# sutro-sh/sutro

Hardware: AMD Instinct MI355X
Metric: output_tokens_per_sec (higher is better)
Workload: dtype bf16; 1 GPU; model=qwen-3-32b, global_batch=2048, seq_len=256, parallelism=dp1, prompt_len=128, priming=seeded

## Files before the change

csrc/bindings.cpp:

```cpp
#include <torch/extension.h>

#include <hip/hip_runtime.h>
#include <c10/hip/HIPStream.h>

#define CHECK_CUDA(x) TORCH_CHECK((x).is_cuda(), #x " must be a GPU tensor")
#define CHECK_CONTIG(x) TORCH_CHECK((x).is_contiguous(), #x " must be contiguous")
#define CHECK_BF16(x) \
  TORCH_CHECK((x).scalar_type() == at::kBFloat16, #x " must be bf16")

static hipStream_t cur_stream() {
  return c10::hip::getCurrentHIPStream().stream();
}

extern "C" {
void sutro_rmsnorm(void*, const void*, const void*, float, long, int,
                   hipStream_t);
void sutro_fused_add_rmsnorm(void*, void*, const void*, float, long, int,
                             hipStream_t);
void sutro_silu_mul(void*, const void*, long, int, hipStream_t);
void sutro_rope_and_cache(void*, void*, const void*, const long*, const long*,
                          void*, void*, const float*, int, int, int, int, int,
                          hipStream_t);
static bool is_fp8(const torch::Tensor& t) {
  return t.scalar_type() == at::kFloat8_e4m3fn;
}
void sutro_mean_pool_normalize(float*, const void*, const int*, int, int,
                               hipStream_t);
void sutro_attn_decode(void*, const void*, const void*, const void*,
                       const int*, const int*, int, int, int, int, int, int,
                       int, float, hipStream_t);
void sutro_attn_prefill(void*, const void*, const void*, const void*,
                        const int*, const int*, const int*, const int*,
                        const int*, int, int, int, int, int, int, float,
                        hipStream_t);
void sutro_attn_decode_shared(void*, const void*, const void*, const void*,
                              const int*, const int*, int, int, int, int,
                              float, int, int, const int*, const int*, int,
                              int, float*, float*, float*, hipStream_t);
int sutro_attn_prefix_tile_rows(int, int);
void sutro_mfma32_probe(float*, const void*, const void*, hipStream_t);
void sutro_gemm_tn_launch(void*, const void*, const void*, const void*, int,
                          int, long, int, int, int, int, hipStream_t);
int sutro_gemm_tn_pipe_launch(void*, const void*, const void*, const void*,
                              int, int, long, int, int, int, hipStream_t);
void sutro_mfma16_probe(float*, const void*, const void*, hipStream_t);
void sutro_hd64_stage_probe(float*, float*, void*, const void*, const void*,
                            const void*, int, float, hipStream_t);
void sutro_qkv_prep(const void*, void*, void*, void*, const long*, const long*,
                    const float*, const void*, const void*, float, int, int,
                    int, int, int, int, int, hipStream_t);
void sutro_sampler_fused(const void*, int, const float*, const float*,
                         const int*, const float*, const unsigned int*, int,
                         long, int, int, int*, float*, hipStream_t);
void sutro_grouped_gemm(void*, const void*, const void*, const int*,
                        const int*, const int*, int, int, int, long, int,
                        int, hipStream_t);
void sutro_moe_combine(void*, const void*, const long*, const float*, int,
                       int, int, hipStream_t);
void sutro_logit_penalties(void*, int, const int*, const int*, const int*,
                           const int*, const int*, const float*, const float*,
                           const float*, const int*, const float*, int, int,
                           long, int, int, int, int, int, hipStream_t);
void sutro_quant_rows_fp8(void*, float*, const void*, const int*, int, long,
                          int, int, hipStream_t);
void sutro_grouped_gemm_fp8(void*, const void*, const float*, const void*,
                            const float*, const int*, const int*, const int*,
                            int, int, int, long, int, int, hipStream_t);
void sutro_quant_weight_mxfp4(void*, void*, const void*, long, int, int,
                              hipStream_t);
void sutro_grouped_gemm_mxfp4(void*, const void*, const float*, const void*,
                              const void*, const int*, const int*, const int*,
                              int, int, int, long, int, int, hipStream_t);
int sutro_gemm_tn_fp8_pipe_launch(void*, const void*, const float*,
                                  const void*, const float*, const void*, int,
                                  int, long, int, int, hipStream_t);
}

void rmsnorm(torch::Tensor out, torch::Tensor x, torch::Tensor w, double eps) {
  CHECK_CUDA(x); CHECK_CONTIG(x); CHECK_BF16(x);
  const long C = x.size(-1);
  const long rows = x.numel() / C;
  TORCH_CHECK(C % 8 == 0 && C <= 16384, "unsupported row size ", C);
  sutro_rmsnorm(out.data_ptr(), x.data_ptr(), w.data_ptr(), (float)eps, rows,
                (int)C, cur_stream());
}

void fused_add_rmsnorm(torch::Tensor x, torch::Tensor residual, torch::Tensor w,
                       double eps) {
  CHECK_CUDA(x); CHECK_CONTIG(x); CHECK_BF16(x); CHECK_CONTIG(residual);
  const long C = x.size(-1);
  const long rows = x.numel() / C;
  TORCH_CHECK(C % 8 == 0 && C <= 16384, "unsupported row size ", C);
  sutro_fused_add_rmsnorm(x.data_ptr(), residual.data_ptr(), w.data_ptr(),
                          (float)eps, rows, (int)C, cur_stream());
}

void silu_mul(torch::Tensor out, torch::Tensor x) {
// ... 137 lines not shown
                 is_fp8(k_cache) ? 1 : 0, cur_stream());
}

torch::Tensor gemm_tn(torch::Tensor x, torch::Tensor w,
                      c10::optional<torch::Tensor> res, long bm, long bn,
                      long swz, long xcd_swz) {
  CHECK_CUDA(x); CHECK_BF16(x); CHECK_CUDA(w); CHECK_BF16(w);
  TORCH_CHECK(x.is_contiguous() && w.is_contiguous(), "contiguous required");
  const long M = x.size(0), K = x.size(1), N = w.size(0);
  TORCH_CHECK(w.size(1) == K, "K mismatch");
  TORCH_CHECK(M % bm == 0 && K % 64 == 0, "shape not tile-divisible");
  auto out = torch::empty({M, N}, x.options());
  const void* rp = nullptr;
  if (res.has_value()) {
    CHECK_CUDA(*res); CHECK_BF16(*res);
    TORCH_CHECK(res->is_contiguous() && res->size(0) == M && res->size(1) == N,
                "res shape");
    rp = res->data_ptr();
  }
  sutro_gemm_tn_launch(out.data_ptr(), x.data_ptr(), w.data_ptr(), rp, (int)M,
                       (int)N, K, (int)bm, (int)bn, (int)swz, (int)xcd_swz,
                       cur_stream());
  return out;
}

torch::Tensor gemm_tn_pipelined(torch::Tensor x, torch::Tensor w,
                                c10::optional<torch::Tensor> res, long swz,
                                long xcd_swz) {
  CHECK_CUDA(x); CHECK_BF16(x); CHECK_CUDA(w); CHECK_BF16(w);
  TORCH_CHECK(x.dim() == 2 && w.dim() == 2, "x and w must be 2-d");
  TORCH_CHECK(x.is_contiguous() && w.is_contiguous(), "contiguous required");
  const long M = x.size(0), K = x.size(1), N = w.size(0);
  TORCH_CHECK(w.size(1) == K, "K mismatch");
  TORCH_CHECK(M >= 1 && N >= 1 && K >= 64 && K % 64 == 0,
              "shape not tile-divisible");
  TORCH_CHECK(M < (1L << 31) && N < (1L << 31), "M/N too large");
  TORCH_CHECK(swz >= 0 && swz <= 2, "swz must be 0, 1 or 2");
  auto out = torch::empty({M, N}, x.options());
  const void* rp = nullptr;
  if (res.has_value()) {
    CHECK_CUDA(*res); CHECK_BF16(*res);
    TORCH_CHECK(res->is_contiguous() && res->dim() == 2 &&
                res->size(0) == M && res->size(1) == N, "res shape");
    rp = res->data_ptr();
  }
  const int e = sutro_gemm_tn_pipe_launch(
      out.data_ptr(), x.data_ptr(), w.data_ptr(), rp, (int)M, (int)N, K,
      rp ? 1 : 0, (int)swz, (int)xcd_swz, cur_stream());
  TORCH_CHECK(e == 0, "gemm_tn_pipelined launch setup failed: ", e);
  return out;
}

torch::Tensor gemm_gate_up_silu(torch::Tensor x, torch::Tensor w, long swz,
                                long xcd_swz) {
  CHECK_CUDA(x); CHECK_BF16(x); CHECK_CUDA(w); CHECK_BF16(w);
  TORCH_CHECK(x.dim() == 2 && w.dim() == 2, "x and w must be 2-d");
  TORCH_CHECK(x.is_contiguous() && w.is_contiguous(), "contiguous required");
  const long M = x.size(0), K = x.size(1), N = w.size(0);
  TORCH_CHECK(w.size(1) == K, "K mismatch");
  TORCH_CHECK(M >= 1 && K >= 64 && K % 64 == 0, "shape not tile-divisible");
  TORCH_CHECK(N >= 256 && N % 256 == 0,
              "gate_up rows must be 2*I with I % 128 == 0");
  TORCH_CHECK(M < (1L << 31) && N < (1L << 31), "M/N too large");
  TORCH_CHECK(swz >= 0 && swz <= 2, "swz must be 0, 1 or 2");
  auto out = torch::empty({M, N / 2}, x.options());
  const int e = sutro_gemm_tn_pipe_launch(
      out.data_ptr(), x.data_ptr(), w.data_ptr(), nullptr, (int)M, (int)N, K,
      2, (int)swz, (int)xcd_swz, cur_stream());
  TORCH_CHECK(e == 0, "gemm_gate_up_silu launch setup failed: ", e);
  return out;
}

static void check_fp8_gemm_args(const torch::Tensor& a_q,
                                const torch::Tensor& a_scale,
                                const torch::Tensor& w_q,
                                const torch::Tensor& w_scale) {
  CHECK_CUDA(a_q); CHECK_CONTIG(a_q); CHECK_CUDA(w_q); CHECK_CONTIG(w_q);
  TORCH_CHECK(is_fp8(a_q) && is_fp8(w_q), "a_q, w_q must be float8_e4m3fn");
  CHECK_CUDA(a_scale); CHECK_CONTIG(a_scale);
  CHECK_CUDA(w_scale); CHECK_CONTIG(w_scale);
  TORCH_CHECK(a_scale.scalar_type() == at::kFloat
              && w_scale.scalar_type() == at::kFloat, "scales must be f32");
  TORCH_CHECK(a_q.dim() == 2 && w_q.dim() == 2, "a_q and w_q must be 2-d");
  const long M = a_q.size(0), Kp = a_q.size(1), N = w_q.size(0);
  TORCH_CHECK(w_q.size(1) == Kp, "Kp mismatch");
  TORCH_CHECK(M >= 1 && Kp >= 128 && Kp % 128 == 0,
              "needs M >= 1 and Kp a positive multiple of 128 (Kp=", Kp, ")");
  TORCH_CHECK(M <= (1L << 31) - 256 && N <= (1L << 31) - 256,
              "M/N too large");
  TORCH_CHECK(a_scale.numel() == M, "a_scale must be [M]");
  TORCH_CHECK(w_scale.numel() == N, "w_scale must be [N]");
}

torch::Tensor gemm_fp8_pipelined(torch::Tensor a_q, torch::Tensor a_scale,
                                 torch::Tensor w_q, torch::Tensor w_scale,
                                 c10::optional<torch::Tensor> res,
                                 long xcd_swz) {
  check_fp8_gemm_args(a_q, a_scale, w_q, w_scale);
  const long M = a_q.size(0), Kp = a_q.size(1), N = w_q.size(0);
  TORCH_CHECK(N >= 64 && N % 64 == 0, "N must be a multiple of 64 (N=", N, ")");
  auto out = torch::empty({M, N}, a_q.options().dtype(at::kBFloat16));
  const void* rp = nullptr;
  if (res.has_value()) {
    CHECK_CUDA(*res); CHECK_BF16(*res);
    TORCH_CHECK(res->is_contiguous() && res->dim() == 2 &&
                res->size(0) == M && res->size(1) == N, "res shape");
    rp = res->data_ptr();
  }
  const int e = sutro_gemm_tn_fp8_pipe_launch(
      out.data_ptr(), a_q.data_ptr(), a_scale.data_ptr<float>(),
      w_q.data_ptr(), w_scale.data_ptr<float>(), rp, (int)M, (int)N, Kp,
      rp ? 1 : 0, (int)xcd_swz, cur_stream());
  TORCH_CHECK(e == 0, "gemm_fp8_pipelined launch setup failed: ", e);
  return out;
}

torch::Tensor gemm_fp8_gate_up_silu(torch::Tensor a_q, torch::Tensor a_scale,
                                    torch::Tensor w_q, torch::Tensor w_scale,
                                    long xcd_swz) {
  check_fp8_gemm_args(a_q, a_scale, w_q, w_scale);
  const long M = a_q.size(0), Kp = a_q.size(1), N = w_q.size(0);
// ... 322 lines not shown
  const long need = 2 * (max_hist_len + n_bias);
  const int log2_cap = need <= 2048 ? 11 : (need <= 8192 ? 13 : 14);
  sutro_logit_penalties(logits.data_ptr(), f32 ? 1 : 0,
                        row_idx.data_ptr<int>(), hist.data_ptr<int>(),
                        slot.data_ptr<int>(), hist_len.data_ptr<int>(),
                        prompt_len.data_ptr<int>(), rep.data_ptr<float>(),
                        pres.data_ptr<float>(), freq.data_ptr<float>(), btp,
                        bvp, (int)m, (int)n, v_row, (int)vl, (int)n_slots,
                        (int)lcap, (int)n_bias, log2_cap, cur_stream());
}

PYBIND11_MODULE(TORCH_EXTENSION_NAME, m) {
  m.def("rmsnorm", &rmsnorm, "RMSNorm (bf16, CDNA4)");
  m.def("fused_add_rmsnorm", &fused_add_rmsnorm, "residual+=x; x=rmsnorm");
  m.def("silu_mul", &silu_mul, "fused SwiGLU");
  m.def("rope_and_cache", &rope_and_cache, "RoPE + paged KV write");
  m.def("qkv_prep", &qkv_prep, "fused qk-norm + RoPE + KV write + q gather");
  m.def("mean_pool_normalize", &mean_pool_normalize, "varlen mean pool + L2");
  m.def("paged_attention", &paged_attention, "paged prefill+decode attention");
  m.def("paged_attention_decode_shared", &paged_attention_decode_shared,
        "decode attention, shared-prefix tiles + per-row continuation");
  m.def("prefix_tile_rows", &prefix_tile_rows,
        "rows per shared-prefix tile for a (Hq, Hk) head layout");
  m.def("mfma32_probe", &mfma32_probe, "MFMA fragment-layout probe");
  m.def("mfma16_probe", &mfma16_probe, "16x16 MFMA fragment-layout probe");
  m.def("hd64_stage_probe", &hd64_stage_probe, "D=64 decode stage dump probe");
  m.def("moe_combine", &moe_combine, "fused MoE weighted gather-combine");
  m.def("grouped_gemm", &grouped_gemm,
        "dropless MoE grouped GEMM (padded segments, static grid)");
  m.def("quant_rows_fp8", &quant_rows_fp8,
        "bf16 rows -> e4m3 codes + f32 per-row scale (K padded to 128)");
  m.def("grouped_gemm_fp8", &grouped_gemm_fp8,
        "dropless MoE grouped GEMM, e4m3 operands on the block-scaled MFMA");
  m.def("quant_weight_mxfp4", &quant_weight_mxfp4,
        "bf16 rows -> e2m1 code pairs + e8m0 scale per 32 (K padded to 128)");
  m.def("grouped_gemm_mxfp4", &grouped_gemm_mxfp4,
        "dropless MoE grouped GEMM, e4m3 x MXFP4 on the block-scaled MFMA");
  m.def("sampler_fused", &sampler_fused,
        "fused mask+temp+topk/topp+sample+logprob (radix descent, no sort)");
  m.def("logit_penalties", &logit_penalties,
        "sparse repetition/presence/frequency penalties + logit_bias "
        "(LDS hash of the row history, in place)");
  m.def("gemm_tn", &gemm_tn, "bf16 TN GEMM (MFMA, glds dbuf)",
        py::arg("x"), py::arg("w"), py::arg("res") = c10::nullopt,
        py::arg("bm") = 256, py::arg("bn") = 256, py::arg("swz") = 2,
        py::arg("xcd_swz") = 0);
  m.def("gemm_tn_pipelined", &gemm_tn_pipelined,
        "bf16 TN GEMM (MFMA, 8-phase glds pipeline, any M/N)",
        py::arg("x"), py::arg("w"), py::arg("res") = c10::nullopt,
        py::arg("swz") = 2, py::arg("xcd_swz") = 1);
  m.def("gemm_gate_up_silu", &gemm_gate_up_silu,
        "SwiGLU fused into the pipelined gate_up GEMM",
        py::arg("x"), py::arg("w"), py::arg("swz") = 2,
        py::arg("xcd_swz") = 1);
  m.def("gemm_fp8_pipelined", &gemm_fp8_pipelined,
        "e4m3 W8A8 TN GEMM (block-scaled MFMA, 8-phase glds pipeline)",
        py::arg("a_q"), py::arg("a_scale"), py::arg("w_q"),
        py::arg("w_scale"), py::arg("res") = c10::nullopt,
        py::arg("xcd_swz") = 1);
  m.def("gemm_fp8_gate_up_silu", &gemm_fp8_gate_up_silu,
        "SwiGLU fused into the pipelined e4m3 gate_up GEMM",
        py::arg("a_q"), py::arg("a_scale"), py::arg("w_q"),
        py::arg("w_scale"), py::arg("xcd_swz") = 1);
}
```

csrc/gemm_tn_pipe.hip:

```cpp
#include "common.h"

typedef s16x8 bf16x8;

namespace {

__device__ __forceinline__ f32x4 mfma16(bf16x8 a, bf16x8 b, f32x4 c) {
  return __builtin_amdgcn_mfma_f32_16x16x32_bf16(a, b, c, 0, 0, 0);
}

__device__ __forceinline__ void glds16(const char* g, char* lds) {
  __builtin_amdgcn_global_load_lds(
      (const __attribute__((address_space(1))) u32*)g,
      (__attribute__((address_space(3))) u32*)lds, 16, 0, 0);
}

template <int SWZ>
__device__ __forceinline__ u32 swz(u32 byte) {
  if (SWZ == 1) return byte ^ (((byte >> 9) & 1u) << 5);
  if (SWZ == 2) return byte ^ (((byte >> 8) & 7u) << 4);
  return byte;
}

constexpr int HT = 16384;
constexpr int KTILE_B = 65536;
constexpr int SLOT_B0 = 0, SLOT_A0 = 1, SLOT_B1 = 2, SLOT_A1 = 3;

struct Src {
  const char* p[2];
};

template <int SWZ>
__device__ __forceinline__ Src make_src(const u16* base, long row0,
                                        long rows_valid, long Kb, int wave,
                                        int lane) {
  Src s;
#pragma unroll
  for (int j = 0; j < 2; ++j) {
    const u32 b = (u32)(wave * 2 + j) * 1024u + (u32)lane * 16u;
    const u32 lb = swz<SWZ>(b);
    long row = (long)(lb >> 7);
    row = row < rows_valid ? row : rows_valid - 1;
    s.p[j] = (const char*)base + (row0 + row) * Kb + (lb & 127u);
  }
  return s;
}

__device__ __forceinline__ void stage_half(char* slot_wave, const Src& s,
                                           long koff) {
  glds16(s.p[0] + koff, slot_wave);
  glds16(s.p[1] + koff, slot_wave + 1024);
}

__device__ __forceinline__ bf16x8 lds_frag(const char* smem, u32 off) {
  return *(const bf16x8*)(smem + off);
}

}

template <int EPI, int SWZ>
__global__ __launch_bounds__(512) void gemm_tn_pipe_kernel(
    u16* __restrict__ out, const u16* __restrict__ x,
    const u16* __restrict__ w, const u16* __restrict__ res, int M, int N,
    long K, int xcd_swz) {
  extern __shared__ __attribute__((aligned(1024))) char smem[];

  const int lane = threadIdx.x & 63;
  const int wave = __builtin_amdgcn_readfirstlane(threadIdx.x >> 6);
  const int wm = wave >> 2;
  const int wn = wave & 3;

  int bid = blockIdx.x;
  if (xcd_swz) {
    const int nwg = gridDim.x;
    const int q = nwg >> 3, r = nwg & 7;
    const int xcd = bid & 7, seq = bid >> 3;
    bid = (xcd < r ? xcd * (q + 1) : r * (q + 1) + (xcd - r) * q) + seq;
  }
  const int MT = (M + 255) >> 8;
  const int m0 = (bid % MT) * 256;
  const int I = N >> 1;
  const int nt = bid / MT;
  const int nb0 = (EPI == 2) ? nt * 128 : nt * 256;
  const int nb1 = (EPI == 2) ? I + nt * 128 : nt * 256 + 128;
  const int nlim = (EPI == 2) ? I : N;

  const long Kb = K * 2;
  const long a0v = min(128, M - m0);
  const long a1v = max(1, min(128, M - m0 - 128));
  const long b0v = min(128, nlim - nb0);
  const long b1v = (EPI == 2) ? 128 : max(1, min(128, N - nb1));
  const long a1r = (M - m0 - 128 >= 1) ? m0 + 128 : m0 + a0v - 1;
  const long b1r = (EPI == 2 || N - nb1 >= 1) ? nb1 : nb0 + b0v - 1;
  const Src sB0 = make_src<SWZ>(w, nb0, b0v, Kb, wave, lane);
  const Src sA0 = make_src<SWZ>(x, m0, a0v, Kb, wave, lane);
  const Src sB1 = make_src<SWZ>(w, b1r, b1v, Kb, wave, lane);
  const Src sA1 = make_src<SWZ>(x, a1r, a1v, Kb, wave, lane);

  char* const sw = smem + wave * 2048;

  u32 aoff[2], boff[2];
#pragma unroll
  for (int kk = 0; kk < 2; ++kk) {
    const u32 kc = (u32)(kk * 4 + (lane >> 4)) * 16u;
    aoff[kk] = swz<SWZ>((u32)(wm * 64 + (lane & 15)) * 128u + kc);
    boff[kk] = swz<SWZ>((u32)(wn * 32 + (lane & 15)) * 128u + kc);
  }

  f32x4 acc[2][2][4][2];
#pragma unroll
  for (int a = 0; a < 2; ++a)
#pragma unroll
    for (int b = 0; b < 2; ++b)
#pragma unroll
      for (int i = 0; i < 4; ++i)
#pragma unroll
        for (int j = 0; j < 2; ++j) acc[a][b][i][j] = f32x4{0.f, 0.f, 0.f, 0.f};

  const int KT = (int)(K >> 6);
  const int klast = KT - 1;

  {
    const long k1 = (long)min(1, klast) * 128;
    stage_half(sw + SLOT_B0 * HT, sB0, 0);
    stage_half(sw + SLOT_A0 * HT, sA0, 0);
    stage_half(sw + SLOT_B1 * HT, sB1, 0);
    stage_half(sw + SLOT_A1 * HT, sA1, 0);
    stage_half(sw + KTILE_B + SLOT_B0 * HT, sB0, k1);
    stage_half(sw + KTILE_B + SLOT_A0 * HT, sA0, k1);
    stage_half(sw + KTILE_B + SLOT_B1 * HT, sB1, k1);
    asm volatile("s_waitcnt vmcnt(6)" ::: "memory");
    __builtin_amdgcn_s_barrier();
    if (wm == 1) __builtin_amdgcn_s_barrier();
  }

  bf16x8 fa[4][2], fb0[2][2], fb1[2][2];

#define PHASE_SYNC_MFMA(A_, B_, FB_)                                     \
  __builtin_amdgcn_sched_barrier(0);                                     \
  __builtin_amdgcn_s_barrier();                                          \
  asm volatile("s_waitcnt lgkmcnt(0)" ::: "memory");                     \
  __builtin_amdgcn_sched_barrier(0);                                     \
  __builtin_amdgcn_s_setprio(1);                                         \
  _Pragma("unroll") for (int kk = 0; kk < 2; ++kk)                       \
  _Pragma("unroll") for (int i = 0; i < 4; ++i)                          \
  _Pragma("unroll") for (int j = 0; j < 2; ++j)                          \
      acc[A_][B_][i][j] = mfma16(fa[i][kk], FB_[j][kk], acc[A_][B_][i][j]); \
  __builtin_amdgcn_s_setprio(0);                                         \
  __builtin_amdgcn_sched_barrier(0);                                     \
  __builtin_amdgcn_s_barrier();                                          \
  __builtin_amdgcn_sched_barrier(0);

#define KTILE(P)                                                         \
  {                                                                      \
    const char* cur = smem + (P) * KTILE_B;                              \
    char* nxt = sw + ((P) ^ 1) * KTILE_B;                                \
    char* own = sw + (P) * KTILE_B;                                      \
                                                                \
    _Pragma("unroll") for (int j = 0; j < 2; ++j)                        \
    _Pragma("unroll") for (int kk = 0; kk < 2; ++kk)                     \
        fb0[j][kk] = lds_frag(cur + SLOT_B0 * HT + j * 2048, boff[kk]);  \
    __builtin_amdgcn_sched_barrier(0);                                   \
    _Pragma("unroll") for (int i = 0; i < 4; ++i)                        \
    _Pragma("unroll") for (int kk = 0; kk < 2; ++kk)                     \
        fa[i][kk] = lds_frag(cur + SLOT_A0 * HT + i * 2048, aoff[kk]);   \
    __builtin_amdgcn_sched_barrier(0);                                   \
    stage_half(nxt + SLOT_A1 * HT, sA1, kn1);                            \
    __builtin_amdgcn_sched_barrier(0);                                   \
    asm volatile("s_waitcnt lgkmcnt(8)" ::: "memory");                   \
    PHASE_SYNC_MFMA(0, 0, fb0)                                           \
                                                                \
    _Pragma("unroll") for (int j = 0; j < 2; ++j)                        \
    _Pragma("unroll") for (int kk = 0; kk < 2; ++kk)                     \
        fb1[j][kk] = lds_frag(cur + SLOT_B1 * HT + j * 2048, boff[kk]);  \
    __builtin_amdgcn_sched_barrier(0);                                   \
    stage_half(own + SLOT_B0 * HT, sB0, kn2);                            \
    PHASE_SYNC_MFMA(0, 1, fb1)                                           \
                                                                \
    _Pragma("unroll") for (int i = 0; i < 4; ++i)                        \
    _Pragma("unroll") for (int kk = 0; kk < 2; ++kk)                     \
        fa[i][kk] = lds_frag(cur + SLOT_A1 * HT + i * 2048, aoff[kk]);   \
    __builtin_amdgcn_sched_barrier(0);                                   \
    stage_half(own + SLOT_A0 * HT, sA0, kn2);                            \
    PHASE_SYNC_MFMA(1, 0, fb0)                                           \
                                                                \
    stage_half(own + SLOT_B1 * HT, sB1, kn2);                            \
    __builtin_amdgcn_sched_barrier(0);                                   \
    asm volatile("s_waitcnt vmcnt(6)" ::: "memory");                     \
    PHASE_SYNC_MFMA(1, 1, fb1)                                           \
  }

  for (int t = 0; t < KT; t += 2) {
    {
      const long kn1 = (long)min(t + 1, klast) * 128;
      const long kn2 = (long)min(t + 2, klast) * 128;
      KTILE(0)
    }
    if (t + 1 < KT) {
      const long kn1 = (long)min(t + 2, klast) * 128;
      const long kn2 = (long)min(t + 3, klast) * 128;
      KTILE(1)
    }
  }
#undef KTILE
#undef PHASE_SYNC_MFMA

  asm volatile("s_waitcnt vmcnt(0)" ::: "memory");
  if (wm == 0) __builtin_amdgcn_s_barrier();

  const int drow = (lane >> 4) * 4;
  const int dcol = lane & 15;
  if (EPI == 2) {
#pragma unroll
    for (int a = 0; a < 2; ++a)
#pragma unroll
      for (int i = 0; i < 4; ++i)
#pragma unroll
        for (int j = 0; j < 2; ++j) {
          const int gn = nb0 + wn * 32 + j * 16 + dcol;
          const int gm = m0 + a * 128 + wm * 64 + i * 16 + drow;
#pragma unroll
          for (int r = 0; r < 4; ++r) {
            if (gm + r >= M) continue;
            const float gf = bf2f(f2bf(acc[a][0][i][j][r]));
            const float uf = bf2f(f2bf(acc[a][1][i][j][r]));
            const float s = gf / (1.f + __expf(-gf));
            out[(long)(gm + r) * I + gn] = f2bf(s * uf);
          }
        }
  } else {
#pragma unroll
    for (int a = 0; a < 2; ++a)
#pragma unroll
      for (int b = 0; b < 2; ++b)
#pragma unroll
        for (int i = 0; i < 4; ++i)
#pragma unroll
          for (int j = 0; j < 2; ++j) {
            const int gn = nb0 + b * 128 + wn * 32 + j * 16 + dcol;
            if (gn >= N) continue;
            const int gm = m0 + a * 128 + wm * 64 + i * 16 + drow;
#pragma unroll
            for (int r = 0; r < 4; ++r) {
              if (gm + r >= M) continue;
              const long o = (long)(gm + r) * N + gn;
              float v = acc[a][b][i][j][r];
              if (EPI == 1) v += bf2f(res[o]);
              out[o] = f2bf(v);
            }
          }
  }
}

extern "C" int sutro_gemm_tn_pipe_launch(void* out, const void* x,
                                         const void* w, const void* res,
                                         int M, int N, long K, int epi,
                                         int swz_mode, int xcd_swz,
                                         hipStream_t stream) {
  constexpr int LDS_BYTES = 2 * KTILE_B;
  const int mt = (M + 255) / 256;
  const int ntl = (epi == 2) ? (N / 2) / 128 : (N + 255) / 256;
  dim3 grid(mt * ntl), block(512);
  constexpr int MAX_DEV = 64;
  static bool attr_set[3][3][MAX_DEV];
  int dev = 0;
  const int ed = (int)hipGetDevice(&dev);
  if (ed != 0) return ed;
#define LAUNCH_1(EPI, SWZ)                                                   \
  if (epi == EPI && swz_mode == SWZ) {                                       \
    if (dev < 0 || dev >= MAX_DEV || !attr_set[EPI][SWZ][dev]) {             \
      const int e = (int)hipFuncSetAttribute(                                \
          (const void*)gemm_tn_pipe_kernel<EPI, SWZ>,                        \
          hipFuncAttributeMaxDynamicSharedMemorySize, LDS_BYTES);            \
      if (e != 0) return e;                                                  \
      if (dev >= 0 && dev < MAX_DEV) attr_set[EPI][SWZ][dev] = true;         \
    }                                                                        \
    gemm_tn_pipe_kernel<EPI, SWZ><<<grid, block, LDS_BYTES, stream>>>(       \
        (u16*)out, (const u16*)x, (const u16*)w, (const u16*)res, M, N, K,   \
        xcd_swz);                                                            \
    return 0;                                                                \
  }
#define LAUNCH(EPI) LAUNCH_1(EPI, 0) LAUNCH_1(EPI, 1) LAUNCH_1(EPI, 2)
  LAUNCH(0)
  LAUNCH(1)
  LAUNCH(2)
#undef LAUNCH
#undef LAUNCH_1
  return -1;
}
```

sutro_amd/ops/__init__.py:

```python

from __future__ import annotations

import os
from typing import Optional

import torch

from . import torch_ref

_C = None
_C_ERR: Optional[str] = None
try:
    from sutro_amd import _C as _C
except Exception as e:
    _C_ERR = f"{type(e).__name__}: {e}"


def hip_available() -> bool:
    return _C is not None


def _require_hip():
    if _C is None:
        raise RuntimeError(
            "sutro_amd HIP extension (_C) is not built but a GPU tensor was passed. "
            "Build it with `python setup.py build_ext --inplace` "
            f"(import error: {_C_ERR})"
        )
    return _C


_FORCE_REF = os.environ.get("SUTRO_AMD_FORCE_TORCH_REF", "0") == "1"


def _use_hip(t: torch.Tensor) -> bool:
    return t.is_cuda and not _FORCE_REF


def rmsnorm(x: torch.Tensor, weight: torch.Tensor, eps: float) -> torch.Tensor:
    if _use_hip(x):
        out = torch.empty_like(x)
        _require_hip().rmsnorm(out, x, weight, eps)
        return out
    return torch_ref.rmsnorm(x, weight, eps)


def fused_add_rmsnorm(x, residual, weight, eps: float):
    if _use_hip(x):
        _require_hip().fused_add_rmsnorm(x, residual, weight, eps)
        return x, residual
    return torch_ref.fused_add_rmsnorm(x, residual, weight, eps)


def silu_mul(x: torch.Tensor) -> torch.Tensor:
    if _use_hip(x):
        T, two_i = x.shape
        out = torch.empty((T, two_i // 2), dtype=x.dtype, device=x.device)
        _require_hip().silu_mul(out, x)
        return out
    return torch_ref.silu_mul(x)


GATE_UP_FUSED_RULE: dict = {
    (5120, 51200): (1152, frozenset({1536, 1664, 1792})),
}

_GATE_UP_FORCE: Optional[bool] = {"1": True, "0": False}.get(
    os.environ.get("SUTRO_GATE_UP_FUSED", ""))


def set_gate_up_fused(mode: Optional[bool]) -> None:
    global _GATE_UP_FORCE
    _GATE_UP_FORCE = mode


def gate_up_silu_qualifies(x: torch.Tensor, weight: torch.Tensor) -> bool:
    return (x.dim() == 2 and weight.dim() == 2 and x.shape[0] >= 1
            and x.dtype == torch.bfloat16 and weight.dtype == torch.bfloat16
            and x.is_contiguous() and weight.is_contiguous()
            and x.shape[1] == weight.shape[1] and x.shape[1] % 64 == 0
            and weight.shape[0] >= 256 and weight.shape[0] % 256 == 0)


def gate_up_silu(x: torch.Tensor, weight: torch.Tensor) -> torch.Tensor:
    if _use_hip(x) and gate_up_silu_qualifies(x, weight):
        if _GATE_UP_FORCE is None:
            min_m, held_back = GATE_UP_FUSED_RULE.get(
                (x.shape[1], weight.shape[0]), (None, ()))
            fused = (min_m is not None and x.shape[0] >= min_m
                     and x.shape[0] not in held_back)
        else:
            fused = _GATE_UP_FORCE
        if fused:
            return _require_hip().gemm_gate_up_silu(x, weight)
    return silu_mul(torch.nn.functional.linear(x, weight))


def fused_qkv_prep(
    qkv: torch.Tensor,
    num_heads: int, num_kv_heads: int, head_dim: int,
    positions: torch.Tensor, slot_mapping: torch.Tensor,
    k_cache: torch.Tensor, v_cache: torch.Tensor,
    cos_sin: torch.Tensor,
    q_norm_w: Optional[torch.Tensor] = None,
    k_norm_w: Optional[torch.Tensor] = None,
    eps: float = 1e-6,
) -> torch.Tensor:
    T = qkv.shape[0]
    if _use_hip(qkv):
        q_out = torch.empty((T, num_heads, head_dim), dtype=qkv.dtype,
                            device=qkv.device)
        _require_hip().qkv_prep(qkv, q_out, k_cache, v_cache, positions,
                                slot_mapping, cos_sin, q_norm_w, k_norm_w, eps)
        return q_out
    q_size = num_heads * head_dim
    kv_size = num_kv_heads * head_dim
    q, k, v = qkv.split([q_size, kv_size, kv_size], dim=-1)
    q = q.reshape(T, num_heads, head_dim).contiguous()
    k = k.reshape(T, num_kv_heads, head_dim).contiguous()
    v = v.reshape(T, num_kv_heads, head_dim).contiguous()
    if q_norm_w is not None:
        q = torch_ref.rmsnorm(q, q_norm_w, eps)
    if k_norm_w is not None:
        k = torch_ref.rmsnorm(k, k_norm_w, eps)
    q, k = torch_ref.apply_rope(q, k, positions, cos_sin)
    torch_ref.write_kv_cache(k, v, k_cache, v_cache, slot_mapping)
    return q


def rope_and_cache(
    q: torch.Tensor, k: torch.Tensor, v: torch.Tensor,
    positions: torch.Tensor, slot_mapping: torch.Tensor,
    k_cache: torch.Tensor, v_cache: torch.Tensor,
    cos_sin: torch.Tensor,
) -> torch.Tensor:
    if _use_hip(q):
        _require_hip().rope_and_cache(q, k, v, positions, slot_mapping,
                                      k_cache, v_cache, cos_sin)
        return q
    q, k = torch_ref.apply_rope(q, k, positions, cos_sin)
    torch_ref.write_kv_cache(k, v, k_cache, v_cache, slot_mapping)
    return q


_EMPTY_I32: Optional[torch.Tensor] = None


# ... 233 lines not shown
```

Before: 7492 tokens/s.

## Add grouped/banded tile ordering and persistent variant to fused SwiGLU gate_up GEMM

```diff
diff --git a/csrc/bindings.cpp b/csrc/bindings.cpp
--- a/csrc/bindings.cpp
+++ b/csrc/bindings.cpp
@@ -42,7 +42,9 @@
 void sutro_gemm_tn_launch(void*, const void*, const void*, const void*, int,
                           int, long, int, int, int, int, hipStream_t);
 int sutro_gemm_tn_pipe_launch(void*, const void*, const void*, const void*,
-                              int, int, long, int, int, int, hipStream_t);
+                              int, int, long, int, int, int, hipStream_t,
+                              int variant = 0, int group_m = 0,
+                              int num_blocks = 0, int wide = 0);
 void sutro_mfma16_probe(float*, const void*, const void*, hipStream_t);
 void sutro_hd64_stage_probe(float*, float*, void*, const void*, const void*,
                             const void*, int, float, hipStream_t);
@@ -286,7 +288,8 @@
 }
 
 torch::Tensor gemm_gate_up_silu(torch::Tensor x, torch::Tensor w, long swz,
-                                long xcd_swz) {
+                                long xcd_swz, long variant, long group_m,
+                                long num_blocks, bool wide) {
   CHECK_CUDA(x); CHECK_BF16(x); CHECK_CUDA(w); CHECK_BF16(w);
   TORCH_CHECK(x.dim() == 2 && w.dim() == 2, "x and w must be 2-d");
   TORCH_CHECK(x.is_contiguous() && w.is_contiguous(), "contiguous required");
@@ -297,10 +300,28 @@
               "gate_up rows must be 2*I with I % 128 == 0");
   TORCH_CHECK(M < (1L << 31) && N < (1L << 31), "M/N too large");
   TORCH_CHECK(swz >= 0 && swz <= 2, "swz must be 0, 1 or 2");
+  TORCH_CHECK(variant == 0 || variant == 1,
+              "variant must be 0 (one tile per block) or 1 (persistent)");
+  TORCH_CHECK(group_m > -(1L << 24) && group_m < (1L << 24),
+              "group_m out of range");
+  TORCH_CHECK(group_m >= 0 || xcd_swz != 0,
+              "the banded tile order (group_m < 0) needs xcd_swz");
+  TORCH_CHECK(num_blocks >= -1 && num_blocks <= (1L << 20),
+              "num_blocks out of range");
+  TORCH_CHECK(((M + 255) / 256) * (N / 256) < (1L << 31), "too many tiles");
+  if (variant == 1) {
+    TORCH_CHECK(K % 128 == 0 && K <= (1L << 23),
+                "the persistent gate_up kernel needs K % 128 == 0 (got K = ",
+                K, "); use variant 0");
+  } else {
+    TORCH_CHECK(num_blocks == 0 && !wide,
+                "num_blocks / wide apply to the persistent variant only");
+  }
   auto out = torch::empty({M, N / 2}, x.options());
   const int e = sutro_gemm_tn_pipe_launch(
       out.data_ptr(), x.data_ptr(), w.data_ptr(), nullptr, (int)M, (int)N, K,
-      2, (int)swz, (int)xcd_swz, cur_stream());
+      2, (int)swz, (int)xcd_swz, cur_stream(), (int)variant, (int)group_m,
+      (int)num_blocks, wide ? 1 : 0);
   TORCH_CHECK(e == 0, "gemm_gate_up_silu launch setup failed: ", e);
   return out;
 }
@@ -729,7 +750,9 @@
   m.def("gemm_gate_up_silu", &gemm_gate_up_silu,
         "SwiGLU fused into the pipelined gate_up GEMM",
         py::arg("x"), py::arg("w"), py::arg("swz") = 2,
-        py::arg("xcd_swz") = 1);
+        py::arg("xcd_swz") = 1, py::arg("variant") = 0,
+        py::arg("group_m") = 0, py::arg("num_blocks") = 0,
+        py::arg("wide") = false);
   m.def("gemm_fp8_pipelined", &gemm_fp8_pipelined,
         "e4m3 W8A8 TN GEMM (block-scaled MFMA, 8-phase glds pipeline)",
         py::arg("a_q"), py::arg("a_scale"), py::arg("w_q"),
diff --git a/csrc/gemm_tn_pipe.hip b/csrc/gemm_tn_pipe.hip
--- a/csrc/gemm_tn_pipe.hip
+++ b/csrc/gemm_tn_pipe.hip
@@ -55,85 +55,90 @@
   return *(const bf16x8*)(smem + off);
 }
 
-}
-
-template <int EPI, int SWZ>
-__global__ __launch_bounds__(512) void gemm_tn_pipe_kernel(
-    u16* __restrict__ out, const u16* __restrict__ x,
-    const u16* __restrict__ w, const u16* __restrict__ res, int M, int N,
-    long K, int xcd_swz) {
-  extern __shared__ __attribute__((aligned(1024))) char smem[];
-
-  const int lane = threadIdx.x & 63;
-  const int wave = __builtin_amdgcn_readfirstlane(threadIdx.x >> 6);
-  const int wm = wave >> 2;
-  const int wn = wave & 3;
-
-  int bid = blockIdx.x;
-  if (xcd_swz) {
-    const int nwg = gridDim.x;
-    const int q = nwg >> 3, r = nwg & 7;
-    const int xcd = bid & 7, seq = bid >> 3;
-    bid = (xcd < r ? xcd * (q + 1) : r * (q + 1) + (xcd - r) * q) + seq;
-  }
-  const int MT = (M + 255) >> 8;
-  const int m0 = (bid % MT) * 256;
-  const int I = N >> 1;
-  const int nt = bid / MT;
-  const int nb0 = (EPI == 2) ? nt * 128 : nt * 256;
-  const int nb1 = (EPI == 2) ? I + nt * 128 : nt * 256 + 128;
-  const int nlim = (EPI == 2) ? I : N;
-
-  const long Kb = K * 2;
-  const long a0v = min(128, M - m0);
-  const long a1v = max(1, min(128, M - m0 - 128));
-  const long b0v = min(128, nlim - nb0);
-  const long b1v = (EPI == 2) ? 128 : max(1, min(128, N - nb1));
+__device__ __forceinline__ void tile_mn(int tile, int MT, int NT, int group_m,
+                                        int& mt, int& nt) {
+  if (group_m <= 0 || group_m >= MT) {
+    mt = tile % MT;
+    nt = tile / MT;
+    return;
+  }
+  const int per = group_m * NT;
+  const int g = tile / per;
+  const int first = g * group_m;
+  const int gsz = min(group_m, MT - first);
+  const int local = tile - g * per;
+  mt = first + local % gsz;
+  nt = local / gsz;
+}
+
+__device__ __forceinline__ void tile_mn_banded(int xl, int i, int nx, int MT,
+                                               int NT, int group_m, int& mt,
+                                               int& nt) {
+  const int a = MT / nx, b = MT - a * nx;
+  const int whole = a * NT;
+  if (i < whole) {
+    tile_mn(i, a, NT, -group_m, mt, nt);
+    mt += a * xl;
+    return;
+  }
+  const int left = b * NT;
+  const int q = left / nx, r = left % nx;
+  const int idx =
+      (xl < r ? xl * (q + 1) : r * (q + 1) + (xl - r) * q) + (i - whole);
+  mt = nx * a + idx % b;
+  nt = idx / b;
+}
+
+struct USrc {
+  const char* base;
+  u32 o0, o1;
+};
+
+template <int SWZ>
+__device__ __forceinline__ void lane_offsets(u32& o0, u32& o1, int rows_valid,
+                                             u32 Kb, int wave, int lane) {
+  u32 o[2];
+#pragma unroll
+  for (int j = 0; j < 2; ++j) {
+    const u32 b = (u32)(wave * 2 + j) * 1024u + (u32)lane * 16u;
+    const u32 lb = swz<SWZ>(b);
+    const u32 row = min(lb >> 7, (u32)(rows_valid - 1));
+    o[j] = row * Kb + (lb & 127u);
+  }
+  o0 = o[0];
+  o1 = o[1];
+}
+
+__device__ __forceinline__ void stage_half(char* slot_wave, const USrc& s,
+                                           long koff) {
+  glds16(s.base + koff + s.o0, slot_wave);
+  glds16(s.base + koff + s.o1, slot_wave + 1024);
+}
+
+struct TileSrc {
+  const char *b0, *a0, *b1, *a1;
+  u32 a0o0, a0o1, a1o0, a1o1;
+};
+
+template <int SWZ>
+__device__ __forceinline__ TileSrc swiglu_tile_src(const u16* x, const u16* w,
+                                                   int M, int I, u32 Kb,
+                                                   int m0, int nb0, int wave,
+                                                   int lane) {
+  const int a0v = min(128, M - m0);
+  const int a1v = max(1, min(128, M - m0 - 128));
   const long a1r = (M - m0 - 128 >= 1) ? m0 + 128 : m0 + a0v - 1;
-  const long b1r = (EPI == 2 || N - nb1 >= 1) ? nb1 : nb0 + b0v - 1;
-  const Src sB0 = make_src<SWZ>(w, nb0, b0v, Kb, wave, lane);
-  const Src sA0 = make_src<SWZ>(x, m0, a0v, Kb, wave, lane);
-  const Src sB1 = make_src<SWZ>(w, b1r, b1v, Kb, wave, lane);
-  const Src sA1 = make_src<SWZ>(x, a1r, a1v, Kb, wave, lane);
-
-  char* const sw = smem + wave * 2048;
-
-  u32 aoff[2], boff[2];
-#pragma unroll
-  for (int kk = 0; kk < 2; ++kk) {
-    const u32 kc = (u32)(kk * 4 + (lane >> 4)) * 16u;
-    aoff[kk] = swz<SWZ>((u32)(wm * 64 + (lane & 15)) * 128u + kc);
-    boff[kk] = swz<SWZ>((u32)(wn * 32 + (lane & 15)) * 128u + kc);
-  }
-
-  f32x4 acc[2][2][4][2];
-#pragma unroll
-  for (int a = 0; a < 2; ++a)
-#pragma unroll
-    for (int b = 0; b < 2; ++b)
-#pragma unroll
-      for (int i = 0; i < 4; ++i)
-#pragma unroll
-        for (int j = 0; j < 2; ++j) acc[a][b][i][j] = f32x4{0.f, 0.f, 0.f, 0.f};
-
-  const int KT = (int)(K >> 6);
-  const int klast = KT - 1;
-
-  {
-    const long k1 = (long)min(1, klast) * 128;
-    stage_half(sw + SLOT_B0 * HT, sB0, 0);
-    stage_half(sw + SLOT_A0 * HT, sA0, 0);
-    stage_half(sw + SLOT_B1 * HT, sB1, 0);
-    stage_half(sw + SLOT_A1 * HT, sA1, 0);
-    stage_half(sw + KTILE_B + SLOT_B0 * HT, sB0, k1);
-    stage_half(sw + KTILE_B + SLOT_A0 * HT, sA0, k1);
-    stage_half(sw + KTILE_B + SLOT_B1 * HT, sB1, k1);
-    asm volatile("s_waitcnt vmcnt(6)" ::: "memory");
-    __builtin_amdgcn_s_barrier();
-    if (wm == 1) __builtin_amdgcn_s_barrier();
-  }
-
-  bf16x8 fa[4][2], fb0[2][2], fb1[2][2];
+  TileSrc t;
+  t.b0 = (const char*)w + (long)nb0 * Kb;
+  t.a0 = (const char*)x + (long)m0 * Kb;
+  t.b1 = (const char*)w + ((long)I + nb0) * Kb;
+  t.a1 = (const char*)x + a1r * Kb;
+  lane_offsets<SWZ>(t.a0o0, t.a0o1, a0v, Kb, wave, lane);
+  lane_offsets<SWZ>(t.a1o0, t.a1o1, a1v, Kb, wave, lane);
+  return t;
+}
+
+}
 
 #define PHASE_SYNC_MFMA(A_, B_, FB_)                                     \
   __builtin_amdgcn_sched_barrier(0);                                     \
@@ -150,44 +155,133 @@
   __builtin_amdgcn_s_barrier();                                          \
   __builtin_amdgcn_sched_barrier(0);
 
-#define KTILE(P)                                                         \
+#define KTILE_G(P, SA1, KA1, SB0, SA0, SB1, K2)                          \
   {                                                                      \
-    const char* cur = smem + (P) * KTILE_B;                              \
-    char* nxt = sw + ((P) ^ 1) * KTILE_B;                                \
-    char* own = sw + (P) * KTILE_B;                                      \
+    const char* kt_cur = smem + (P) * KTILE_B;                           \
+    char* kt_nxt = sw + ((P) ^ 1) * KTILE_B;                             \
+    char* kt_own = sw + (P) * KTILE_B;                                   \
                                                                 \
     _Pragma("unroll") for (int j = 0; j < 2; ++j)                        \
     _Pragma("unroll") for (int kk = 0; kk < 2; ++kk)                     \
-        fb0[j][kk] = lds_frag(cur + SLOT_B0 * HT + j * 2048, boff[kk]);  \
+        fb0[j][kk] = lds_frag(kt_cur + SLOT_B0 * HT + j * 2048,       \
+                              boff[kk]);                                 \
     __builtin_amdgcn_sched_barrier(0);                                   \
     _Pragma("unroll") for (int i = 0; i < 4; ++i)                        \
     _Pragma("unroll") for (int kk = 0; kk < 2; ++kk)                     \
-        fa[i][kk] = lds_frag(cur + SLOT_A0 * HT + i * 2048, aoff[kk]);   \
+        fa[i][kk] = lds_frag(kt_cur + SLOT_A0 * HT + i * 2048,        \
+                             aoff[kk]);                                  \
     __builtin_amdgcn_sched_barrier(0);                                   \
-    stage_half(nxt + SLOT_A1 * HT, sA1, kn1);                            \
+    stage_half(kt_nxt + SLOT_A1 * HT, SA1, KA1);                         \
     __builtin_amdgcn_sched_barrier(0);                                   \
     asm volatile("s_waitcnt lgkmcnt(8)" ::: "memory");                   \
     PHASE_SYNC_MFMA(0, 0, fb0)                                           \
                                                                 \
     _Pragma("unroll") for (int j = 0; j < 2; ++j)                        \
     _Pragma("unroll") for (int kk = 0; kk < 2; ++kk)                     \
-        fb1[j][kk] = lds_frag(cur + SLOT_B1 * HT + j * 2048, boff[kk]);  \
+        fb1[j][kk] = lds_frag(kt_cur + SLOT_B1 * HT + j * 2048,       \
+                              boff[kk]);                                 \
     __builtin_amdgcn_sched_barrier(0);                                   \
-    stage_half(own + SLOT_B0 * HT, sB0, kn2);                            \
+    stage_half(kt_own + SLOT_B0 * HT, SB0, K2);                          \
     PHASE_SYNC_MFMA(0, 1, fb1)                                           \
                                                                 \
     _Pragma("unroll") for (int i = 0; i < 4; ++i)                        \
     _Pragma("unroll") for (int kk = 0; kk < 2; ++kk)                     \
-        fa[i][kk] = lds_frag(cur + SLOT_A1 * HT + i * 2048, aoff[kk]);   \
+        fa[i][kk] = lds_frag(kt_cur + SLOT_A1 * HT + i * 2048,        \
+                             aoff[kk]);                                  \
     __builtin_amdgcn_sched_barrier(0);                                   \
-    stage_half(own + SLOT_A0 * HT, sA0, kn2);                            \
+    stage_half(kt_own + SLOT_A0 * HT, SA0, K2);                          \
     PHASE_SYNC_MFMA(1, 0, fb0)                                           \
                                                                 \
-    stage_half(own + SLOT_B1 * HT, sB1, kn2);                            \
+    stage_half(kt_own + SLOT_B1 * HT, SB1, K2);                          \
     __builtin_amdgcn_sched_barrier(0);                                   \
     asm volatile("s_waitcnt vmcnt(6)" ::: "memory");                     \
     PHASE_SYNC_MFMA(1, 1, fb1)                                           \
   }
+
+template <int EPI, int SWZ>
+__global__ __launch_bounds__(512) void gemm_tn_pipe_kernel(
+    u16* __restrict__ out, const u16* __restrict__ x,
+    const u16* __restrict__ w, const u16* __restrict__ res, int M, int N,
+    long K, int xcd_swz, int group_m) {
+  extern __shared__ __attribute__((aligned(1024))) char smem[];
+
+  const int lane = threadIdx.x & 63;
+  const int wave = __builtin_amdgcn_readfirstlane(threadIdx.x >> 6);
+  const int wm = wave >> 2;
+  const int wn = wave & 3;
+
+  int bid = blockIdx.x;
+  if (xcd_swz) {
+    const int nwg = gridDim.x;
+    const int q = nwg >> 3, r = nwg & 7;
+    const int xcd = bid & 7, seq = bid >> 3;
+    bid = (xcd < r ? xcd * (q + 1) : r * (q + 1) + (xcd - r) * q) + seq;
+  }
+  const int MT = (M + 255) >> 8;
+  const int I = N >> 1;
+  int mt, nt;
+  if (group_m < 0)
+    tile_mn_banded(blockIdx.x & 7, blockIdx.x >> 3, 8, MT,
+                   (int)gridDim.x / MT, group_m, mt, nt);
+  else
+    tile_mn(bid, MT, (int)gridDim.x / MT, group_m, mt, nt);
+  const int m0 = mt * 256;
+  const int nb0 = (EPI == 2) ? nt * 128 : nt * 256;
+  const int nb1 = (EPI == 2) ? I + nt * 128 : nt * 256 + 128;
+  const int nlim = (EPI == 2) ? I : N;
+
+  const long Kb = K * 2;
+  const long a0v = min(128, M - m0);
+  const long a1v = max(1, min(128, M - m0 - 128));
+  const long b0v = min(128, nlim - nb0);
+  const long b1v = (EPI == 2) ? 128 : max(1, min(128, N - nb1));
+  const long a1r = (M - m0 - 128 >= 1) ? m0 + 128 : m0 + a0v - 1;
+  const long b1r = (EPI == 2 || N - nb1 >= 1) ? nb1 : nb0 + b0v - 1;
+  const Src sB0 = make_src<SWZ>(w, nb0, b0v, Kb, wave, lane);
+  const Src sA0 = make_src<SWZ>(x, m0, a0v, Kb, wave, lane);
+  const Src sB1 = make_src<SWZ>(w, b1r, b1v, Kb, wave, lane);
+  const Src sA1 = make_src<SWZ>(x, a1r, a1v, Kb, wave, lane);
+
+  char* const sw = smem + wave * 2048;
+
+  u32 aoff[2], boff[2];
+#pragma unroll
+  for (int kk = 0; kk < 2; ++kk) {
+    const u32 kc = (u32)(kk * 4 + (lane >> 4)) * 16u;
+    aoff[kk] = swz<SWZ>((u32)(wm * 64 + (lane & 15)) * 128u + kc);
+    boff[kk] = swz<SWZ>((u32)(wn * 32 + (lane & 15)) * 128u + kc);
+  }
+
+  f32x4 acc[2][2][4][2];
+#pragma unroll
+  for (int a = 0; a < 2; ++a)
+#pragma unroll
+    for (int b = 0; b < 2; ++b)
+#pragma unroll
+      for (int i = 0; i < 4; ++i)
+#pragma unroll
+        for (int j = 0; j < 2; ++j) acc[a][b][i][j] = f32x4{0.f, 0.f, 0.f, 0.f};
+
+  const int KT = (int)(K >> 6);
+  const int klast = KT - 1;
+
+  {
+    const long k1 = (long)min(1, klast) * 128;
+    stage_half(sw + SLOT_B0 * HT, sB0, 0);
+    stage_half(sw + SLOT_A0 * HT, sA0, 0);
+    stage_half(sw + SLOT_B1 * HT, sB1, 0);
+    stage_half(sw + SLOT_A1 * HT, sA1, 0);
+    stage_half(sw + KTILE_B + SLOT_B0 * HT, sB0, k1);
+    stage_half(sw + KTILE_B + SLOT_A0 * HT, sA0, k1);
+    stage_half(sw + KTILE_B + SLOT_B1 * HT, sB1, k1);
+    asm volatile("s_waitcnt vmcnt(6)" ::: "memory");
+    __builtin_amdgcn_s_barrier();
+    if (wm == 1) __builtin_amdgcn_s_barrier();
+  }
+
+  bf16x8 fa[4][2], fb0[2][2], fb1[2][2];
+
+#define KTILE(P) KTILE_G(P, sA1, kn1, sB0, sA0, sB1, kn2)
 
   for (int t = 0; t < KT; t += 2) {
     {
@@ -202,7 +296,6 @@
     }
   }
 #undef KTILE
-#undef PHASE_SYNC_MFMA
 
   asm volatile("s_waitcnt vmcnt(0)" ::: "memory");
   if (wm == 0) __builtin_amdgcn_s_barrier();
@@ -251,16 +344,217 @@
   }
 }
 
+template <int SWZ, bool WIDE>
+__global__ __launch_bounds__(512) void gemm_swiglu_persist_kernel(
+    u16* __restrict__ out, const u16* __restrict__ x,
+    const u16* __restrict__ w, int M, int N, long K, int xcd_swz,
+    int group_m) {
+  extern __shared__ __attribute__((aligned(1024))) char smem[];
+
+  const int lane = threadIdx.x & 63;
+  const int wave = __builtin_amdgcn_readfirstlane(threadIdx.x >> 6);
+  const int wm = wave >> 2;
+  const int wn = wave & 3;
+
+  const int I = N >> 1;
+  const int MT = (M + 255) >> 8;
+  const int NT = I >> 7;
+  const int tiles = MT * NT;
+
+  const int nb = gridDim.x;
+  const int nx = xcd_swz ? min(8, nb) : 1;
+  const int xl = blockIdx.x % nx, slot = blockIdx.x / nx;
+  const int slots = (nb - xl + nx - 1) / nx;
+  const int q = tiles / nx, r = tiles % nx;
+  const int span0 = xl < r ? xl * (q + 1) : r * (q + 1) + (xl - r) * q;
+  const int span_n = q + (xl < r ? 1 : 0);
+  if (slot >= span_n) return;
+  const int cnt = (span_n - slot + slots - 1) / slots;
+
+  const u32 Kb = (u32)K * 2u;
+  const int KT = (int)(K >> 6);
+  const long klb = (long)(KT - 1) * 128;
+  u32 bo0, bo1;
+  lane_offsets<SWZ>(bo0, bo1, 128, Kb, wave, lane);
+
+  int mt, nt;
+#define TILE_AT(IDX)                                                     \
+  if (group_m < 0)                                                       \
+    tile_mn_banded(xl, (IDX), nx, MT, NT, group_m, mt, nt);              \
+  else                                                                   \
+    tile_mn(span0 + (IDX), MT, NT, group_m, mt, nt);
+  TILE_AT(slot)
+  int m0 = mt * 256, nb0 = nt * 128;
+  TileSrc cur = swiglu_tile_src<SWZ>(x, w, M, I, Kb, m0, nb0, wave, lane);
+
+  char* const sw = smem + wave * 2048;
+
+  u32 aoff[2], boff[2];
+#pragma unroll
+  for (int kk = 0; kk < 2; ++kk) {
+    const u32 kc = (u32)(kk * 4 + (lane >> 4)) * 16u;
+    aoff[kk] = swz<SWZ>((u32)(wm * 64 + (lane & 15)) * 128u + kc);
+    boff[kk] = swz<SWZ>((u32)(wn * 32 + (lane & 15)) * 128u + kc);
+  }
+
+  f32x4 acc[2][2][4][2];
+#pragma unroll
+  for (int a = 0; a < 2; ++a)
+#pragma unroll
+    for (int b = 0; b < 2; ++b)
+#pragma unroll
+      for (int i = 0; i < 4; ++i)
+#pragma unroll
+        for (int j = 0; j < 2; ++j) acc[a][b][i][j] = f32x4{0.f, 0.f, 0.f, 0.f};
+
+#define S_B0(T) (USrc{T.b0, bo0, bo1})
+#define S_A0(T) (USrc{T.a0, T.a0o0, T.a0o1})
+#define S_B1(T) (USrc{T.b1, bo0, bo1})
+#define S_A1(T) (USrc{T.a1, T.a1o0, T.a1o1})
+  stage_half(sw + SLOT_B0 * HT, S_B0(cur), 0);
+  stage_half(sw + SLOT_A0 * HT, S_A0(cur), 0);
+  stage_half(sw + SLOT_B1 * HT, S_B1(cur), 0);
+  stage_half(sw + SLOT_A1 * HT, S_A1(cur), 0);
+  stage_half(sw + KTILE_B + SLOT_B0 * HT, S_B0(cur), 128);
+  stage_half(sw + KTILE_B + SLOT_A0 * HT, S_A0(cur), 128);
+  stage_half(sw + KTILE_B + SLOT_B1 * HT, S_B1(cur), 128);
+  asm volatile("s_waitcnt vmcnt(6)" ::: "memory");
+  __builtin_amdgcn_s_barrier();
+  if (wm == 1) __builtin_amdgcn_s_barrier();
+
+  bf16x8 fa[4][2], fb0[2][2], fb1[2][2];
+
+  const int drow = (lane >> 4) * 4;
+  const int dcol = lane & 15;
+  char* const ep = smem + 2 * KTILE_B + wave * 4096;
+
+  for (int it = 0; it < cnt; ++it) {
+    for (int t = 0; t < KT - 2; t += 2) {
+      const long k1 = (long)(t + 1) * 128;
+      KTILE_G(0, S_A1(cur), k1, S_B0(cur), S_A0(cur), S_B1(cur), k1 + 128)
+      KTILE_G(1, S_A1(cur), k1 + 128, S_B0(cur), S_A0(cur), S_B1(cur),
+              k1 + 256)
+    }
+    const bool more = it + 1 < cnt;
+    TILE_AT(slot + (more ? it + 1 : it) * slots)
+    const int m0n = mt * 256, nb0n = nt * 128;
+    const TileSrc nx_ =
+        swiglu_tile_src<SWZ>(x, w, M, I, Kb, m0n, nb0n, wave, lane);
+    const long kz0 = more ? 0 : klb, kz1 = more ? 128 : klb;
+    KTILE_G(0, S_A1(cur), klb, S_B0(nx_), S_A0(nx_), S_B1(nx_), kz0)
+    KTILE_G(1, S_A1(nx_), kz0, S_B0(nx_), S_A0(nx_), S_B1(nx_), kz1)
+    if (!more) asm volatile("s_waitcnt vmcnt(0)" ::: "memory");
+
+#pragma unroll
+    for (int a = 0; a < 2; ++a) {
+#pragma unroll
+      for (int i = 0; i < 4; ++i)
+#pragma unroll
+        for (int j = 0; j < 2; ++j) {
+          const int gn = nb0 + wn * 32 + j * 16 + dcol;
+          const int gm = m0 + a * 128 + wm * 64 + i * 16 + drow;
+#pragma unroll
+          for (int rr = 0; rr < 4; ++rr) {
+            const float gf = bf2f(f2bf(acc[a][0][i][j][rr]));
+            const float uf = bf2f(f2bf(acc[a][1][i][j][rr]));
+            const float s = gf / (1.f + __expf(-gf));
+            const u16 v = f2bf(s * uf);
+            if (WIDE) {
+              const u32 row = (u32)(i * 16 + drow + rr);
+              const u32 col = (u32)(j * 16 + dcol);
+              *(u16*)(ep + row * 64u + ((((col >> 3) ^ (row >> 2)) & 3u) << 4) +
+                      (col & 7u) * 2u) = v;
+            } else if (gm + rr < M) {
+              out[(long)(gm + rr) * I + gn] = v;
+            }
+            acc[a][0][i][j][rr] = 0.f;
+            acc[a][1][i][j][rr] = 0.f;
+          }
+        }
+      if (WIDE) {
+#pragma unroll
+        for (int p = 0; p < 4; ++p) {
+          const u32 row = (u32)(p * 16 + (lane >> 2));
+          const u32 ch = (u32)(lane & 3);
+          const u32x4 v =
+              *(const u32x4*)(ep + row * 64u + (((ch ^ (row >> 2)) & 3u) << 4));
+          const int gm = m0 + a * 128 + wm * 64 + (int)row;
+          if (gm < M)
+            *(u32x4*)(out + (long)gm * I + nb0 + wn * 32 + ch * 8) = v;
+        }
+      }
+    }
+    cur = nx_;
+    m0 = m0n;
+    nb0 = nb0n;
+  }
+  if (wm == 0) __builtin_amdgcn_s_barrier();
+}
+
+#undef TILE_AT
+#undef S_B0
+#undef S_A0
+#undef S_B1
+#undef S_A1
+#undef KTILE_G
+#undef PHASE_SYNC_MFMA
+
 extern "C" int sutro_gemm_tn_pipe_launch(void* out, const void* x,
                                          const void* w, const void* res,
                                          int M, int N, long K, int epi,
                                          int swz_mode, int xcd_swz,
-                                         hipStream_t stream) {
+                                         hipStream_t stream, int variant,
+                                         int group_m, int num_blocks,
+                                         int wide) {
   constexpr int LDS_BYTES = 2 * KTILE_B;
+  constexpr int MAX_DEV = 64;
   const int mt = (M + 255) / 256;
   const int ntl = (epi == 2) ? (N / 2) / 128 : (N + 255) / 256;
   dim3 grid(mt * ntl), block(512);
-  constexpr int MAX_DEV = 64;
+  if (group_m < 0 && !xcd_swz) return -4;
+  if (variant == 1) {
+    if (epi != 2 || K < 128 || K % 128 != 0 || K > (1L << 23)) return -2;
+    int dev = 0;
+    const int ed = (int)hipGetDevice(&dev);
+    if (ed != 0) return ed;
+    const bool slot_ok = dev >= 0 && dev < MAX_DEV;
+    if (num_blocks < 0) {
+      num_blocks = mt * ntl;
+    } else if (num_blocks == 0) {
+      static int cus[MAX_DEV];
+      int n = slot_ok ? cus[dev] : 0;
+      if (n == 0) {
+        const int e = (int)hipDeviceGetAttribute(
+            &n, hipDeviceAttributeMultiprocessorCount, dev);
+        if (e != 0) return e;
+        if (n <= 0) return -3;
+        if (slot_ok) cus[dev] = n;
+      }
+      num_blocks = n;
+    }
+    static bool pattr_set[3][2][MAX_DEV];
+#define LAUNCH_P(SWZ, WIDE)                                                  \
+  if (swz_mode == SWZ && (wide != 0) == WIDE) {                              \
+    constexpr int LDS_P = LDS_BYTES + (WIDE ? 8 * 4096 : 0);                 \
+    if (!slot_ok || !pattr_set[SWZ][WIDE][dev]) {                            \
+      const int e = (int)hipFuncSetAttribute(                                \
+          (const void*)gemm_swiglu_persist_kernel<SWZ, WIDE>,                \
+          hipFuncAttributeMaxDynamicSharedMemorySize, LDS_P);                \
+      if (e != 0) return e;                                                  \
+      if (slot_ok) pattr_set[SWZ][WIDE][dev] = true;                         \
+    }                                                                        \
+    gemm_swiglu_persist_kernel<SWZ, WIDE>                                    \
+        <<<dim3(num_blocks), block, LDS_P, stream>>>(                        \
+            (u16*)out, (const u16*)x, (const u16*)w, M, N, K, xcd_swz,       \
+            group_m);                                                        \
+    return 0;                                                                \
+  }
+    LAUNCH_P(0, false) LAUNCH_P(1, false) LAUNCH_P(2, false)
+    LAUNCH_P(0, true) LAUNCH_P(1, true) LAUNCH_P(2, true)
+#undef LAUNCH_P
+    return -1;
+  }
+  if (variant != 0) return -1;
   static bool attr_set[3][3][MAX_DEV];
   int dev = 0;
   const int ed = (int)hipGetDevice(&dev);
@@ -276,7 +570,7 @@
     }                                                                        \
     gemm_tn_pipe_kernel<EPI, SWZ><<<grid, block, LDS_BYTES, stream>>>(       \
         (u16*)out, (const u16*)x, (const u16*)w, (const u16*)res, M, N, K,   \
-        xcd_swz);                                                            \
+        xcd_swz, group_m);                                                   \
     return 0;                                                                \
   }
 #define LAUNCH(EPI) LAUNCH_1(EPI, 0) LAUNCH_1(EPI, 1) LAUNCH_1(EPI, 2)
diff --git a/sutro_amd/ops/__init__.py b/sutro_amd/ops/__init__.py
--- a/sutro_amd/ops/__init__.py
+++ b/sutro_amd/ops/__init__.py
@@ -72,6 +72,48 @@
 def set_gate_up_fused(mode: Optional[bool]) -> None:
     global _GATE_UP_FORCE
     _GATE_UP_FORCE = mode
+
+
+GATE_UP_VARIANT_RULE: dict = {
+    (5120, 51200): [(8192, 32768, 0, -8, False)],
+}
+_V1 = (0, 0, False)
+
+
+def _parse_variant(text: str):
+    parts = [p.strip() for p in text.split(",")]
+    if parts[0] == "v1" and len(parts) == 1:
+        return _V1
+    if parts[0] == "persistent" and len(parts) <= 3:
+        group_m = int(parts[1]) if len(parts) > 1 and parts[1] else 0
+        wide = len(parts) > 2 and parts[2] == "wide"
+        if len(parts) > 2 and parts[2] not in ("", "wide"):
+            raise ValueError(f"bad gate_up variant {text!r}")
+        return (1, group_m, wide)
+    raise ValueError(f"bad gate_up variant {text!r}: expected 'v1' or "
+                     "'persistent[,group_m[,wide]]'")
+
+
+_GATE_UP_VARIANT_FORCE = (
+    _parse_variant(os.environ["SUTRO_GATE_UP_VARIANT"])
+    if os.environ.get("SUTRO_GATE_UP_VARIANT") else None)
+
+
+def set_gate_up_variant(mode) -> None:
+    global _GATE_UP_VARIANT_FORCE
+    _GATE_UP_VARIANT_FORCE = None if mode is None else _parse_variant(mode)
+
+
+def gate_up_variant(k: int, two_i: int, m: int):
+    if k % 128 != 0:
+        return _V1
+    if _GATE_UP_VARIANT_FORCE is not None:
+        return _GATE_UP_VARIANT_FORCE
+    for lo, hi, variant, group_m, wide in GATE_UP_VARIANT_RULE.get(
+            (k, two_i), ()):
+        if m >= lo and (hi is None or m <= hi):
+            return (variant, group_m, wide)
+    return _V1
 
 
 def gate_up_silu_qualifies(x: torch.Tensor, weight: torch.Tensor) -> bool:
@@ -92,7 +134,11 @@
         else:
             fused = _GATE_UP_FORCE
         if fused:
-            return _require_hip().gemm_gate_up_silu(x, weight)
+            v = gate_up_variant(x.shape[1], weight.shape[0], x.shape[0])
+            if v == _V1:
+                return _require_hip().gemm_gate_up_silu(x, weight)
+            return _require_hip().gemm_gate_up_silu(
+                x, weight, 2, 1, v[0], v[1], 0, v[2])
     return silu_mul(torch.nn.functional.linear(x, weight))
 
 
```

Result: faster. 7621 tokens/s (median of 6 runs) (+1.7%).
